# zai-org/SCAIL

Measured on AMD Instinct MI355X. Metric: denoising-step latent tokens/sec, higher is better.
Workload: dtype bf16

## Files before the change

include/scail_dit.h:

```cpp
#ifndef SCAIL_DIT_H
#define SCAIL_DIT_H

#include "scail_hip.h"

#ifdef __cplusplus
extern "C" {
#endif

typedef struct scail_dit_config {
    int32_t hidden_size;
    int32_t num_heads;
    int32_t inner_hidden_size;
    int32_t num_layers;
    int32_t text_dim;
    int32_t clip_dim;
    int32_t time_freq_dim;
    int32_t time_embed_dim;
    float layernorm_epsilon;
} scail_dit_config;

typedef struct scail_dit_layer {
    const scail_bf16* qkv_w; const float* qkv_b;
    const scail_bf16* o_w; const float* o_b;
    const float* qn; const float* kn;
// ... 11 lines not shown
    const scail_bf16* time0_w; const float* time0_b;
    const scail_bf16* time2_w; const float* time2_b;
    const scail_bf16* adaln_w; const float* adaln_b;
    const float* adaln_tables;
    const float* final_table;
    const scail_bf16* final_w; const float* final_b;
    const scail_dit_layer* layers;
} scail_dit_weights;

typedef struct scail_dit_cond {
    const scail_bf16* k_text;
    const scail_bf16* vt_text;
    const scail_bf16* k_clip;
    const scail_bf16* vt_clip;
    int64_t Lt, Lc, Bc;
} scail_dit_cond;

typedef struct scail_dit scail_dit;

int scail_dit_create(const scail_dit_config* cfg, const scail_dit_weights* w, scail_dit** out);
void scail_dit_destroy(scail_dit* h);

int64_t scail_dit_workspace_bytes(const scail_dit* h, int64_t B, int64_t T, int64_t H, int64_t W);

#define SCAIL_DIT_CFG_PAIR 1u
int scail_dit_step(scail_dit* h, const float* x, const float* timesteps, const scail_dit_cond* cond,
                   const scail_bf16* ref, int64_t n_ref, const scail_bf16* pose, int64_t n_pose,
                   const float* rope_cos, const float* rope_sin, float* out,
                   int64_t B, int64_t T, int64_t H, int64_t W, uint32_t flags, void* workspace, int64_t workspace_bytes, void* stream);

// ... 100 lines not shown
```

include/scail_hip.h:

```cpp
#ifndef SCAIL_HIP_H
#define SCAIL_HIP_H

#include <stdint.h>

#ifdef __cplusplus
extern "C" {
#endif

typedef uint16_t scail_bf16;

const char* scail_last_error(void);
int scail_abi_version(void);

enum {
    SCAIL_EPI_BIAS = 0,
    SCAIL_EPI_GELU_TANH = 1,
    SCAIL_EPI_GELU_ERF = 2,
    SCAIL_EPI_RESID = 3
};

int scail_gemm_bf16(const scail_bf16* x, int64_t lda, const scail_bf16* w, const float* bias,
                    scail_bf16* y, int64_t ldc, int64_t M, int64_t N, int64_t K, int epilogue,
                    const scail_bf16* resid, int64_t ldr, const float* gate, int64_t gate_stride,
                    int64_t rows_per_batch, void* stream);
// ... 56 lines not shown

int scail_flash_attn_rows_for(int64_t n_batch, int64_t heads, int64_t Lq);

int scail_flash_attn_count_restarts(uint32_t* device_counter);

int scail_cross_attn2_kernel_for(int64_t q_rs, int64_t k1_rs, int64_t k2_rs, int64_t o_rs, int64_t Lq, int64_t Lk1, int64_t Lk2,
                                 int64_t n_batch, int64_t heads);
int scail_cross_attn2_kernel_name_for(int64_t q_rs, int64_t k1_rs, int64_t k2_rs, int64_t o_rs, int64_t Lq, int64_t Lk1, int64_t Lk2,
                                      int64_t n_batch, int64_t heads, char* buf, int64_t len, int64_t* workgroups);
int scail_cross_attn2_bf16(const scail_bf16* q, int64_t q_bs, int64_t q_rs,
                           const scail_bf16* k1, int64_t k1_bs, int64_t k1_rs, const scail_bf16* vt1, int64_t vt1_bs, int64_t Lk1,
                           const scail_bf16* k2, int64_t k2_bs, int64_t k2_rs, const scail_bf16* vt2, int64_t vt2_bs, int64_t Lk2,
                           scail_bf16* o, int64_t o_bs, int64_t o_rs,
                           int64_t n_batch, int64_t heads, int64_t Lq, float scale, void* stream);

int scail_timestep_embedding(const float* t, float* out, int64_t n, int64_t dim, void* stream);

int scail_small_linear(const float* x, const scail_bf16* w, const float* b, float* y, int64_t M,
                       int64_t N, int64_t K, int act_in, int act_out, void* stream);

int scail_adaln_table(const float* emb, const float* table, float* out, int64_t n_layers,
                      int64_t n_batch, int64_t width, void* stream);

int scail_patchify(const float* x, const scail_bf16* ref, const scail_bf16* pose, scail_bf16* tok,
                   int64_t n_batch, int64_t n_ref, int64_t n_pose, int64_t T, int64_t H, int64_t W,
                   int64_t kpad, void* stream);

int scail_patchify_chars(const float* x, const scail_bf16* ref, const scail_bf16* pose, scail_bf16* tok,
                         int64_t n_batch, int64_t n_ref, int64_t n_pose, int64_t n_char, int64_t T, int64_t H, int64_t W,
                         int64_t kpad, void* stream);
// ... 98 lines not shown
```

scail_amd/csrc/attn.hip:

```cpp
#include <algorithm>
#include <atomic>
#include <cstring>
#include "common.h"

#define HD 128
#define QBLK 256
#define KVBLK 64
#define ATT_THREADS 512
#define K_LD (HD + 8)
#define V_LD (KVBLK + 8)
#define ATT_LDS_BYTES (2 * (KVBLK * K_LD + HD * V_LD) * 2)
#define ATT_PP_LDS_BYTES (ATT_LDS_BYTES + QBLK * K_LD * 2)

struct AttnParams {
    const u16* q; int64_t q_bs, q_rs;
    const u16* k; int64_t k_ss, k_bs, k_rs;
    const u16* vt; int64_t vt_ss, vt_bs;
    u16* o; int64_t o_bs, o_rs;
    int heads, Lq, Lk, Lkp, n_seg;
    float sl2;
    int accumulate;
    int probe;
};

// ... 243 lines not shown
    }
    if (p.probe && tid == 0) {
        atomicAdd(&g_attn_clk[0], (unsigned long long)__builtin_amdgcn_s_memtime() - clk0);
        atomicAdd(&g_attn_clk[1], 1ull);
    }
}


struct Cross2Params {
    const u16* q; int64_t q_bs, q_rs;
    const u16* k0; int64_t k0_bs, k0_rs; const u16* vt0; int64_t vt0_bs; int Lk0, Lkp0;
    const u16* k1; int64_t k1_bs, k1_rs; const u16* vt1; int64_t vt1_bs; int Lk1, Lkp1;
    u16* o; int64_t o_bs, o_rs;
    int heads, Lq;
    float sl2;
};

#define X2_THREADS 256
#define X2_LDS_BYTES (2 * (KVBLK * HD + HD * KVBLK) * 2)
__global__ __launch_bounds__(X2_THREADS, 2) void cross_attn2_kernel(Cross2Params p) {
    extern __shared__ __attribute__((aligned(16))) u16 smem[];
    u16* Ks = smem;
    u16* Vs = smem + 2 * KVBLK * HD;

    const int tid = threadIdx.x, lane = tid & 63;
    const int wave = __builtin_amdgcn_readfirstlane(tid >> 6);
    const int ql = lane & 31, g = lane >> 5;
    const int h = blockIdx.y;
    const int64_t b = blockIdx.z;
    const int q0 = blockIdx.x * 128 + wave * 32;

    bf16x8 qf[HD / 16];
    {
        const int qrow = min(q0 + ql, p.Lq - 1);
        const u16* qp = p.q + b * p.q_bs + (int64_t)qrow * p.q_rs + (int64_t)h * HD + g * 8;
#pragma unroll
        for (int ks = 0; ks < HD / 16; ++ks) qf[ks] = *reinterpret_cast<const bf16x8*>(qp + ks * 16);
    }

    const int dk_row = lane >> 4, dk_c = lane & 15, dv_row = lane >> 3, dv_c = lane & 7;
    const u16* kb0 = p.k0 + b * p.k0_bs + (int64_t)h * HD;
    const u16* kb1 = p.k1 + b * p.k1_bs + (int64_t)h * HD;
    const u16* vb0 = p.vt0 + b * p.vt0_bs + (int64_t)h * HD * p.Lkp0;
    const u16* vb1 = p.vt1 + b * p.vt1_bs + (int64_t)h * HD * p.Lkp1;
    const int n0 = p.Lkp0 / KVBLK, n1 = p.Lkp1 / KVBLK, ntiles = n0 + n1;
#define X2_ISSUE(tt_, buf_)                                                                                 \
    {                                                                                                       \
        const bool s1_ = (tt_) >= n0;                                                                       \
        const int key0_ = ((tt_) - (s1_ ? n0 : 0)) * KVBLK;                                                 \
        const u16* kp_ = s1_ ? kb1 : kb0;                                                                   \
        const int64_t krs_ = s1_ ? p.k1_rs : p.k0_rs;                                                       \
        const int last_ = (s1_ ? p.Lk1 : p.Lk0) - 1;                                                        \
        const int lkp_ = s1_ ? p.Lkp1 : p.Lkp0;                                                             \
        const u16* vp_ = (s1_ ? vb1 : vb0) + key0_;                                                         \
        _Pragma("unroll") for (int i_ = 0; i_ < 4; ++i_) {                                                  \
            const int j_ = wave * 4 + i_;                                                                   \
            const int kr_ = 4 * j_ + dk_row;                                                                \
            const u16* ks_src = kp_ + (int64_t)min(key0_ + kr_, last_) * krs_ + ((dk_c ^ (kr_ & 15)) << 3); \
            __builtin_amdgcn_global_load_lds((const __attribute__((address_space(1))) void*)ks_src,          \
                (__attribute__((address_space(3))) void*)(Ks + ((buf_) * KVBLK + 4 * j_) * HD), 16, 0, 0);   \
            const int vr_ = 8 * j_ + dv_row;                                                                \
            const u16* vs_src = vp_ + (int64_t)vr_ * lkp_ + ((dv_c ^ ((vr_ >> 1) & 7)) << 3);               \
            __builtin_amdgcn_global_load_lds((const __attribute__((address_space(1))) void*)vs_src,          \
                (__attribute__((address_space(3))) void*)(Vs + ((buf_) * HD + 8 * j_) * KVBLK), 16, 0, 0);   \
        }                                                                                                   \
    }
    int koff[HD / 16], voff[4];
// ... 36 lines not shown
        for (int f = 0; f < 2; ++f)
#pragma unroll
            for (int e = 0; e < 16; ++e) s[f][e] = 0.f;
        const u16* ks_ = Ks + (cur * KVBLK + ql) * HD;
#pragma unroll
        for (int ks = 0; ks < HD / 16; ++ks) {
#pragma unroll
            for (int f = 0; f < 2; ++f) {
                const bf16x8 kf = *reinterpret_cast<const bf16x8*>(ks_ + f * 32 * HD + koff[ks]);
                s[f] = __builtin_amdgcn_mfma_f32_32x32x16_bf16(kf, qf[ks], s[f], 0, 0, 0);
            }
        }
        {
            const bool s1 = tt >= n0;
            const int t = tt - (s1 ? n0 : 0), ns = s1 ? n1 : n0;
            const int tail = (s1 ? p.Lk1 : p.Lk0) - (ns - 1) * KVBLK;
            if (t == ns - 1 && tail < KVBLK) {
#pragma unroll
                for (int f = 0; f < 2; ++f)
#pragma unroll
                    for (int r = 0; r < 16; ++r) {
                        const int key = 32 * f + (r & 3) + 8 * (r >> 2) + 4 * g;
                        if (key >= tail) s[f][r] = -INFINITY;
                    }
            }
        }
        float mx = s[0][0];
#pragma unroll
        for (int f = 0; f < 2; ++f)
#pragma unroll
            for (int r = 0; r < 16; ++r) mx = fmaxf(mx, s[f][r]);
// ... 685 lines not shown
    return cross_choose(q_rs, k1_rs, k2_rs, o_rs, Lq, Lk1, Lk2, n_batch, heads, false).generated ? 4 : 2;
}

extern "C" int scail_cross_attn2_kernel_name_for(int64_t q_rs, int64_t k1_rs, int64_t k2_rs, int64_t o_rs, int64_t Lq, int64_t Lk1, int64_t Lk2,
                                                 int64_t n_batch, int64_t heads, char* buf, int64_t len, int64_t* workgroups) {
    SCAIL_REQUIRE(buf != nullptr, "null argument");
    SCAIL_REQUIRE(n_batch >= 1 && heads >= 1 && Lq >= 1 && Lk1 >= 1 && Lk2 >= 1, "need at least one pair, one query and one key per set");
    const CrossChoice c = cross_choose(q_rs, k1_rs, k2_rs, o_rs, Lq, Lk1, Lk2, n_batch, heads, workgroups != nullptr);
    if (c.grid < 0) return 2;
    SCAIL_REQUIRE((int64_t)std::strlen(c.name) < len, "buffer too small");
    std::strcpy(buf, c.name);
    if (workgroups != nullptr) *workgroups = c.grid;
    return 0;
}

extern "C" int scail_cross_attn2_bf16(const scail_bf16* q, int64_t q_bs, int64_t q_rs,
                                      const scail_bf16* k1, int64_t k1_bs, int64_t k1_rs, const scail_bf16* vt1, int64_t vt1_bs, int64_t Lk1,
                                      const scail_bf16* k2, int64_t k2_bs, int64_t k2_rs, const scail_bf16* vt2, int64_t vt2_bs, int64_t Lk2,
                                      scail_bf16* o, int64_t o_bs, int64_t o_rs,
                                      int64_t n_batch, int64_t heads, int64_t Lq, float scale, void* stream) {
    SCAIL_REQUIRE(Lk1 >= 1 && Lk2 >= 1 && Lk1 < (1ll << 30) && Lk2 < (1ll << 30), "cross_attn2: each key set needs at least one key");
    SCAIL_REQUIRE(heads >= 1 && heads < 65536 && n_batch < 65536 && Lq < (1ll << 31) - 256, "cross_attn2: grid limits");
    SCAIL_REQUIRE(q_rs % 8 == 0 && k1_rs % 8 == 0 && k2_rs % 8 == 0 && o_rs % 4 == 0 && q_bs % 8 == 0 && k1_bs % 8 == 0 && k2_bs % 8 == 0 &&
                      vt1_bs % 8 == 0 && vt2_bs % 8 == 0 && o_bs % 4 == 0,
                  "cross_attn2: strides must keep 16-byte (q, k, vt) / 8-byte (o) alignment");
    SCAIL_REQUIRE((reinterpret_cast<uintptr_t>(q) & 15) == 0 && (reinterpret_cast<uintptr_t>(k1) & 15) == 0 && (reinterpret_cast<uintptr_t>(k2) & 15) == 0 &&
                      (reinterpret_cast<uintptr_t>(vt1) & 15) == 0 && (reinterpret_cast<uintptr_t>(vt2) & 15) == 0 && (reinterpret_cast<uintptr_t>(o) & 7) == 0,
                  "cross_attn2: pointer alignment");
    if (n_batch == 0 || Lq == 0) return 0;
    const bool prescaled = scale == SCAIL_ATTN_Q_PRESCALED;
    SCAIL_REQUIRE(prescaled || (scale > 0.0f && scale < 3.0e38f), "cross_attn2: scale must be a positive finite number or SCAIL_ATTN_Q_PRESCALED");
    const CrossChoice c = cross_choose(q_rs, k1_rs, k2_rs, o_rs, Lq, Lk1, Lk2, n_batch, heads, true);
    if (c.generated) {
        hipFunction_t fn;
        if (int rc = scail_module_function("attn4", k_attn4_hsaco, c.name, &fn)) return rc;
// ... 3 lines not shown
        a.base.sl2 = prescaled ? 0.0f : scale * 1.4426950408889634f;
        a.base.thr = g_attn4_thr_log2;
        a.base.restarts = nullptr;
        a.k2 = k2; a.vt2 = vt2; a.k2_bs = k2_bs; a.vt2_bs = vt2_bs; a.Lk2 = (int32_t)Lk2; a.Lkp2 = (int32_t)((Lk2 + 63) / 64 * 64);
        a.n_wgs = (int32_t)c.grid;
        a.pad = 0;
        return scail_module_launch("cross_attn2 (attn4_x2)", fn, (unsigned)a.n_wgs, 256, a, stream);
    }
    Cross2Params p;
    p.q = q; p.q_bs = q_bs; p.q_rs = q_rs;
    p.k0 = k1; p.k0_bs = k1_bs; p.k0_rs = k1_rs; p.vt0 = vt1; p.vt0_bs = vt1_bs; p.Lk0 = (int)Lk1; p.Lkp0 = (int)((Lk1 + KVBLK - 1) / KVBLK * KVBLK);
    p.k1 = k2; p.k1_bs = k2_bs; p.k1_rs = k2_rs; p.vt1 = vt2; p.vt1_bs = vt2_bs; p.Lk1 = (int)Lk2; p.Lkp1 = (int)((Lk2 + KVBLK - 1) / KVBLK * KVBLK);
    p.o = o; p.o_bs = o_bs; p.o_rs = o_rs;
    p.heads = (int)heads; p.Lq = (int)Lq;
    p.sl2 = prescaled ? 1.0f : scale * 1.44269504088896340736f;
    const dim3 grid((unsigned)((Lq + 127) / 128), (unsigned)heads, (unsigned)n_batch);
    return scail_launch_lds<cross_attn2_kernel>("cross_attn2", X2_LDS_BYTES, grid, dim3(X2_THREADS), X2_LDS_BYTES, stream, p);
}
```

scail_amd/csrc/dit_step.hip:

```cpp
#include <algorithm>
#include <array>
#include <cmath>
#include <vector>

#include "common.h"
int scail_attn4_preload();
void scail_attn4_rows_hint(int rows);
int scail_gemm4_preload();
#include "../../include/scail_dit.h"

constexpr int PROF_CATS = 5;
struct ProfPool {
    std::vector<hipEvent_t> ev;
    size_t used = 0;
};

struct scail_dit {
    scail_dit_config cfg;
    scail_dit_weights w;
    std::vector<scail_dit_layer> layers;
    bool prof = false;
    ProfPool pool[PROF_CATS];
    hipEvent_t sp_ev[3] = {nullptr, nullptr, nullptr};
    uint32_t* restart_ctr = nullptr;
// ... 263 lines not shown
                           void* stream) {
    const scail_dit_config& c = h->cfg;
    const int64_t D = c.hidden_size, FF = c.inner_hidden_size, nh = c.num_heads;
    const float eps = c.layernorm_epsilon;
    const int64_t Ltp = (cond->Lt + 63) / 64 * 64, Lcp = (cond->Lc + 63) / 64 * 64;
    const int64_t M = nb * rpb;
    const scail_dit_layer& lw = h->layers[i];
    DIT_TRY(scail_layernorm_affine(hid, D, xn, D, lw.ln_w, lw.ln_b, M, D, eps, stream));
    DIT_PROF(SCAIL_DIT_PROF_GEMM, dit_gemm(h, i, G_CQ, bf, xn, D, lw.cq_b, q3, 3 * D, M, D, D, SCAIL_EPI_BIAS, nullptr, 0, nullptr, 0, 0, stream));
    DIT_TRY(scail_rmsnorm_rope_scaled(q3, 3 * D, q3, 3 * D, lw.cqn, nullptr, nullptr, M, M, D, 128, eps, ATTN_LOG2_SCALE, stream));
    const bool shared_clip = cond->Bc == 1;
    const scail_bf16* kt = cond->k_text + (i * Btot + b0) * cond->Lt * D;
    const scail_bf16* vtt = cond->vt_text + (i * Btot + b0) * nh * 128 * Ltp;
    const scail_bf16* kc = cond->k_clip + (i * cond->Bc + (shared_clip ? 0 : b0)) * cond->Lc * D;
    const scail_bf16* vtc = cond->vt_clip + (i * cond->Bc + (shared_clip ? 0 : b0)) * nh * 128 * Lcp;
    DIT_PROF(SCAIL_DIT_PROF_CROSS_ATTN, scail_cross_attn2_bf16(q3, rpb * 3 * D, 3 * D, kt, cond->Lt * D, D, vtt, nh * 128 * Ltp, cond->Lt,
                                                               kc, shared_clip ? 0 : cond->Lc * D, D, vtc, shared_clip ? 0 : nh * 128 * Lcp, cond->Lc,
                                                               att, rpb * D, D, nb, nh, rpb, SCAIL_ATTN_Q_PRESCALED, stream));
    DIT_PROF(SCAIL_DIT_PROF_GEMM, dit_gemm(h, i, G_CO, bf, att, D, lw.co_b, hid, D, M, D, D, SCAIL_EPI_RESID, hid, D, nullptr, 0, 0, stream));
    DIT_TRY(scail_ln_modulate(hid, D, xn, D, m + 3 * D, m + 4 * D, 6 * D, nb, rpb, rpb, 0, D, eps, stream));
    DIT_PROF(SCAIL_DIT_PROF_GEMM, dit_gemm(h, i, G_W1, bf, xn, D, lw.b1, ff, FF, M, FF, D, SCAIL_EPI_GELU_TANH, nullptr, 0, nullptr, 0, 0, stream));
    DIT_PROF(SCAIL_DIT_PROF_GEMM, dit_gemm(h, i, G_W2, bf, ff, FF, lw.b2, hid, D, M, D, FF, SCAIL_EPI_RESID, hid, D, m + 5 * D, 6 * D, rpb, stream));
    return 0;
}
static int block_tail(scail_dit* h, int64_t i, scail_bf16* hid, const float* m, const scail_dit_cond* cond, int64_t B, int64_t Ltok,
                      const BlockBufs& bf, int64_t row0, int64_t rows, bool pair, void* stream) {
    const int64_t D = h->cfg.hidden_size;
    scail_bf16 *att = bf.att, *q = bf.qkv, *xn = bf.xn, *ff = bf.ff;
    if (pair) {
        DIT_TRY(block_attn_out(h, i, hid + row0 * D, att + row0 * D, m, 1, rows, bf, stream));
        if (hipMemcpyAsync(hid + Ltok * D, hid, (size_t)Ltok * D * 2, hipMemcpyDeviceToDevice, (hipStream_t)stream) != hipSuccess) {
            scail_set_error("scail_dit (cfg pair): hipMemcpyAsync failed");
            return 2;
// ... 647 lines not shown
```

scail_amd/csrc/rowops.hip:

```cpp
#include "common.h"
#include <algorithm>
#include <atomic>
#include <cstring>

#define ROW_THREADS 256
#define ROW_MAXV 3

template <int MODE>
__global__ __launch_bounds__(ROW_THREADS) void ln_kernel(
    const u16* __restrict__ x, int64_t ldx, u16* __restrict__ y, int64_t ldy,
    const float* __restrict__ p0, const float* __restrict__ p1, int64_t mod_stride,
    int64_t rows_out, int64_t src_rows_per_batch, int64_t src_row_offset, int D, float eps) {
    __shared__ float red[4];
    const int64_t r = blockIdx.x;
    const int64_t b = r / rows_out;
    const int64_t i = r - b * rows_out;
    const u16* xr = x + (b * src_rows_per_batch + src_row_offset + i) * ldx;
    u16* yr = y + r * ldy;
    const int nvec = D >> 3;
    float v[ROW_MAXV][8];
    float s = 0.f;
#pragma unroll
    for (int j = 0; j < ROW_MAXV; ++j) {
        const int c = threadIdx.x + j * ROW_THREADS;
// ... 1044 lines not shown
    if (n == 0) return 0;
    hipLaunchKernelGGL(mul_bf16_kernel, dim3((unsigned)((n / 8 + 255) / 256)), dim3(256), 0, (hipStream_t)stream, a, b, y, n / 8);
    return scail_check_launch("mul_bf16");
}

extern "C" int scail_row_affine(const scail_bf16* x, scail_bf16* y, const float* rowscale, const scail_bf16* addrow, int64_t add_rows,
                                int64_t rows, int64_t D, void* stream) {
    SCAIL_REQUIRE(D % 8 == 0, "D must be a multiple of 8");
    if (rows == 0) return 0;
    const int64_t total = rows * (D / 8);
    hipLaunchKernelGGL(row_affine_kernel, dim3((unsigned)((total + 255) / 256)), dim3(256), 0, (hipStream_t)stream, x, y, rowscale,
                       addrow, add_rows > 0 ? add_rows : 1, rows, (int)(D / 8));
    return scail_check_launch("row_affine");
}

__global__ __launch_bounds__(256) void comm_standin_kernel(const uint4* __restrict__ src, uint4* __restrict__ dst, int64_t n16, int64_t min_ticks) {
    const int64_t t0 = (int64_t)wall_clock64();
    for (int64_t i = (int64_t)blockIdx.x * 256 + threadIdx.x; i < n16; i += (int64_t)gridDim.x * 256) dst[i] = src[i];
    while ((int64_t)wall_clock64() - t0 < min_ticks) __builtin_amdgcn_s_sleep(64);
}
extern "C" int scail_comm_standin(const void* src, void* dst, int64_t bytes, int32_t workgroups, int64_t min_ns, void* stream) {
    SCAIL_REQUIRE(bytes >= 0 && bytes % 16 == 0 && aligned16(src) && aligned16(dst), "bytes must be a multiple of 16, pointers 16-byte aligned");
    SCAIL_REQUIRE(workgroups >= 1 && workgroups <= 4096 && min_ns >= 0 && min_ns <= 1000000000ll, "workgroups in [1, 4096], min_ns in [0, 1e9]");
    hipLaunchKernelGGL(comm_standin_kernel, dim3((unsigned)workgroups), dim3(256), 0, (hipStream_t)stream,
                       reinterpret_cast<const uint4*>(src), reinterpret_cast<uint4*>(dst), bytes / 16, min_ns / 10);
    return scail_check_launch("comm_standin");
}
```

scail_amd/cstep.py:

```python
from __future__ import annotations

import ctypes as C
from typing import Dict

import torch

from . import lib as L

_p, _i64 = C.c_void_p, C.c_int64


class DitConfig(C.Structure):
    _fields_ = [("hidden_size", C.c_int32), ("num_heads", C.c_int32), ("inner_hidden_size", C.c_int32),
                ("num_layers", C.c_int32), ("text_dim", C.c_int32), ("clip_dim", C.c_int32),
                ("time_freq_dim", C.c_int32), ("time_embed_dim", C.c_int32), ("layernorm_epsilon", C.c_float)]


_LAYER_FIELDS = ["qkv_w", "qkv_b", "o_w", "o_b", "qn", "kn", "cq_w", "cq_b", "co_w", "co_b", "cqn", "ln_w", "ln_b",
                 "w1", "b1", "w2", "b2"]


class DitLayer(C.Structure):
    _fields_ = [(n, _p) for n in _LAYER_FIELDS]


class DitWeights(C.Structure):
    _fields_ = [(n, _p) for n in ("patch_w", "patch_b", "pose_w", "pose_b", "time0_w", "time0_b", "time2_w", "time2_b",
                                  "adaln_w", "adaln_b", "adaln_tables", "final_table", "final_w", "final_b")] + \
               [("layers", C.POINTER(DitLayer))]


class DitCond(C.Structure):
    _fields_ = [("k_text", _p), ("vt_text", _p), ("k_clip", _p), ("vt_clip", _p), ("Lt", _i64), ("Lc", _i64), ("Bc", _i64)]


EXCHANGE_FN = C.CFUNCTYPE(C.c_int, C.c_void_p, C.c_int32, C.c_int32, C.c_int32, C.c_void_p)
SP_ALLGATHER, SP_ULYSSES = 0, 1
SP_FWD_START, SP_FWD_WAIT, SP_BACK_START, SP_BACK_WAIT = 0, 1, 2, 3


class DitSp(C.Structure):
    _fields_ = [("ranks", C.c_int32), ("mode", C.c_int32), ("send", _p), ("recv", _p), ("ofull", _p), ("back", _p),
                ("exchange", EXCHANGE_FN), ("user", _p), ("side_stream", _p * 2)]


def _cond_struct(cond: Dict) -> "DitCond":
    k_text, k_clip = cond["k_text"], cond["k_clip"]
    return DitCond(k_text.data_ptr(), cond["vt_text"].data_ptr(), k_clip.data_ptr(), cond["vt_clip"].data_ptr(),
                   k_text.shape[2], k_clip.shape[2], k_clip.shape[1])


class CStep:

    def __init__(self, net, W: Dict):
        L.load()
        self._keep = W
        cfg = DitConfig(net.hidden_size, net.num_attention_heads, net.inner_hidden_size, net.num_layers, net.text_dim,
                        1280, net.time_freq_dim, net.time_embed_dim, float(net.layernorm_epsilon))
        layers = (DitLayer * net.num_layers)()
        for i, lw in enumerate(W["layers"]):
            for n in _LAYER_FIELDS:
                setattr(layers[i], n, lw[n].data_ptr())
        w = DitWeights(W["patch_w"].data_ptr(), W["patch_b"].data_ptr(), W["pose_w"].data_ptr(), W["pose_b"].data_ptr(),
                       W["time_embed.0.w"].data_ptr(), W["time_embed.0.b"].data_ptr(),
# ... 196 lines not shown
```

scail_amd/dit.py:

```python
from __future__ import annotations

import os

import math
from functools import reduce
from operator import mul
from typing import Dict, Optional

import torch
from torch import nn

from . import lib as L
from . import ops, rope

_STR2DTYPE = {"fp32": torch.float32, "fp16": torch.float16, "bf16": torch.bfloat16}


def _get(args, name, default=None):
    if args is None:
        return default
    if isinstance(args, dict):
        return args.get(name, default)
    return getattr(args, name, default)

# ... 166 lines not shown
        self.gemm_precision, self.fp8_mask = _fp8_options(gemm_precision, fp8_gemms)
        self.fp8_scaling = _fp8_scaling_option(fp8_scaling, self.gemm_precision)
        self.fp8_layer_masks = _fp8_layer_options(fp8_layers, num_layers, self.fp8_mask)
        self.fp8_probe_table = None
        if self.fp8_mask:
            D, FF = self.hidden_size, self.inner_hidden_size
            for name, (n, k) in (("qkv", (3 * D, D)), ("o", (D, D)), ("cq", (D, D)), ("co", (D, D)), ("w1", (FF, D)), ("w2", (D, FF))):
                if self.fp8_mask & L.FP8_GEMMS[name] and (n % 128 or k % 128):
                    raise NotImplementedError(f"fp8 GEMM {name} ({n} x {k}): the fp8 kernel needs N and K multiples of 128")
        self._build_params(device, init_seed)
        self._prepared: Optional[Dict] = None
        self._cond_cache = None
        self._rope_cache: Dict = {}
        self._ws: Dict = {}
        self.cache_conditioning = True
        self.sp = None
        self._tap = None
        self.kernel_timer = None
        self.use_c_step = os.environ.get("SCAIL_C_STEP", "1") != "0"
        self._cstep = None
        self._c_blocks = False

    def param_spec(self) -> Dict[str, tuple]:
        D, FF, Dt = self.hidden_size, self.inner_hidden_size, self.time_embed_dim
        s: Dict[str, tuple] = {}
        s["mixins.patch_embed.proj.weight"] = (D, 20, 1, 2, 2)
        s["mixins.patch_embed.proj.bias"] = (D,)
        s["mixins.patch_embed.proj_pose.weight"] = (D, 20, 1, 2, 2)
        s["mixins.patch_embed.proj_pose.bias"] = (D,)
        for i in range(self.num_layers):
# ... 166 lines not shown
        Ltp, Lcp = (Lt + 63) // 64 * 64, (Lc + 63) // 64 * 64
        nl = self.num_layers
        k_text = torch.empty(nl, B, Lt, D, device=dev, dtype=torch.bfloat16)
        vt_text = torch.empty(nl, B, H, 128, Ltp, device=dev, dtype=torch.bfloat16)
        k_clip = torch.empty(nl, Bc, Lc, D, device=dev, dtype=torch.bfloat16)
        vt_clip = torch.empty(nl, Bc, H, 128, Lcp, device=dev, dtype=torch.bfloat16)
        kv = torch.empty(B, Lt, 2 * D, device=dev, dtype=torch.bfloat16)
        kvc = torch.empty(Bc, Lc, 2 * D, device=dev, dtype=torch.bfloat16)
        for i, lw in enumerate(W["layers"]):
            ops.gemm(text, lw["ckv_w"], lw["ckv_b"], out=kv)
            ops.rmsnorm_rope(kv[..., :D], lw["ckn"], out=k_text[i], eps=self.layernorm_epsilon)
            ops.transpose_v(kv[..., D:], H, out=vt_text[i])
            ops.gemm(cl, lw["clipkv_w"], lw["clipkv_b"], out=kvc)
            ops.rmsnorm_rope(kvc[..., :D], lw["clipkn"], out=k_clip[i], eps=self.layernorm_epsilon)
            ops.transpose_v(kvc[..., D:], H, out=vt_clip[i])
        return dict(k_text=k_text, vt_text=vt_text, k_clip=k_clip, vt_clip=vt_clip)

    def _timed(self, tag, fn, *a, **k):
        if self.kernel_timer is None:
            return fn(*a, **k)
        return self.kernel_timer.run(tag, fn, *a, **k)

    def _rope(self, T, Hp, Wp, H_shift, W_shift, device, n_char=1):
        key = (T, Hp, Wp, H_shift, W_shift, n_char)
        if key not in self._rope_cache:
            mt = (self.num_frames - 1) // self.time_compressed_rate + 1
            cos, sin = rope.build_tables(self.head_dim, T, Hp, Wp, H_shift, W_shift, self.global_rope_H,
                                         self.global_rope_W, max_T=mt, max_H=self.latent_height // 2,
                                         max_W=self.latent_width // 2 + 120, n_char=n_char)
            self._rope_cache[key] = (cos.to(device), sin.to(device))
        return self._rope_cache[key]
# ... 172 lines not shown
            sh_m, sc_m, g_m = m[:, 3 * D:4 * D], m[:, 4 * D:5 * D], m[:, 5 * D:6 * D]
            ops.ln_modulate(h, sh_a, sc_a, out=xn, eps=eps)
            if sp is None:
                ops.gemm(xn, lw["qkv_w"], lw["qkv_b"], out=qkv)
                ops.rmsnorm_rope(k, lw["kn"], cos, sin, rows_per_batch=Ltok, eps=eps)
                ops.transpose_v(v, nh, out=vt)
                ops.rmsnorm_rope(q, lw["qn"], cos, sin, rows_per_batch=Ltok, eps=eps, out_scale=ops.ATTN_LOG2_SCALE)
                self._timed("self_attn", ops.flash_attn, q, k, vt, out=att, q_prescaled=True)
            else:
                sp.self_attention(self, lw, xn, qkv, vt, cos, sin, att, Ltok, eps)
            ops.gemm(att, lw["o_w"], lw["o_b"], out=h, epilogue=L.EPI_RESID, resid=h, gate=g_a, rows_per_batch=Ltok)
            ops.layernorm_affine(h, lw["ln_w"], lw["ln_b"], out=xn, eps=eps)
            cq = qkv[..., :D]
            ops.gemm(xn, lw["cq_w"], lw["cq_b"], out=cq)
            ops.rmsnorm_rope(cq, lw["cqn"], eps=eps, out_scale=ops.ATTN_LOG2_SCALE)
            ops.cross_attn2(cq, cond["k_text"][i], cond["vt_text"][i], cond["k_clip"][i], cond["vt_clip"][i], out=att, q_prescaled=True)
            ops.gemm(att, lw["co_w"], lw["co_b"], out=h, epilogue=L.EPI_RESID, resid=h)
            ops.ln_modulate(h, sh_m, sc_m, out=xn, eps=eps)
            ops.gemm(xn, lw["w1"], lw["b1"], out=ff, epilogue=L.EPI_GELU_TANH)
            ops.gemm(ff, lw["w2"], lw["b2"], out=h, epilogue=L.EPI_RESID, resid=h, gate=g_m, rows_per_batch=Ltok)
            if self._tap is not None:
                self._tap(i, h)

        ops.ln_modulate(h, fin[:, :D], fin[:, D:], out=ws["xf"], eps=eps, rows_out=Lnoise, src_row_offset=Lref)
        ops.gemm(ws["xf"], W["final_w"], W["final_b"], out=ws["tokout"])
        return ops.unpatchify(ws["tokout"], T, H, Wd)
```

scail_amd/lib.py:

```python
from __future__ import annotations

import ctypes as C
import os

_HERE = os.path.dirname(os.path.abspath(__file__))
LIB_PATH = os.path.join(_HERE, "libscail_hip_abl.so" if os.environ.get("SCAIL_ABLATIONS", "0") not in ("", "0") else "libscail_hip.so")

_p = C.c_void_p
_i64 = C.c_int64
_i = C.c_int
_f = C.c_float

SIGNATURES = {
    "scail_gemm_bf16": [_p, _i64, _p, _p, _p, _i64, _i64, _i64, _i64, _i, _p, _i64, _p, _i64, _i64, _p],
    "scail_ln_modulate": [_p, _i64, _p, _i64, _p, _p, _i64, _i64, _i64, _i64, _i64, _i64, _f, _p],
    "scail_layernorm_affine": [_p, _i64, _p, _i64, _p, _p, _i64, _i64, _f, _p],
    "scail_rmsnorm_rope": [_p, _i64, _p, _i64, _p, _p, _p, _i64, _i64, _i64, _i64, _f, _p],
    "scail_rmsnorm_rope_scaled": [_p, _i64, _p, _i64, _p, _p, _p, _i64, _i64, _i64, _i64, _f, _f, _p],
    "scail_rmsnorm_rope_slabs": [_p, _i64, _p, _i64, _i64, _i64, _p, _p, _p, _i64, _i64, _i64, _i64, _f, _f, _p],
    "scail_row_kernel_name_for": [_i, _i64, _i64, _i64, _i64, _p, _i64, _p],
    "scail_slabs_to_rows": [_p, _i64, _i64, _p, _i64, _i64, _i64, _p],
    "scail_transpose_v": [_p, _i64, _i64, _p, _i64, _i64, _i64, _i64, _p],
    "scail_flash_attn_bf16": [_p, _i64, _i64, _p, _i64, _i64, _i64, _p, _i64, _i64, _p, _i64, _i64,
                              _i64, _i64, _i64, _i64, _i64, _f, _i, _p],
    "scail_flash_attn_kernel_for": [_i64, _i64, _i64, _i64, _i64, _i, _i],
    "scail_flash_attn_kernel_name_for": [_i64, _i64, _i64, _i64, _i64, _i64, _i64, _i, _i, _p, _i64, _p],
    "scail_flash_attn_rows_for": [_i64, _i64, _i64],
    "scail_flash_attn_count_restarts": [_p],
    "scail_comm_standin": [_p, _p, _i64, C.c_int32, _i64, _p],
    "scail_cross_attn2_kernel_for": [_i64, _i64, _i64, _i64, _i64, _i64, _i64, _i64, _i64],
    "scail_cross_attn2_kernel_name_for": [_i64, _i64, _i64, _i64, _i64, _i64, _i64, _i64, _i64, _p, _i64, _p],
    "scail_gemm_kernel_for": [_i64, _i64, _i64, _i64, _i64, _i64, _i],
    "scail_gemm_kernel_name_for": [_i64, _i64, _i64, _i64, _i64, _i64, _i, _i, _p, _i64],
    "scail_conv3d_kernel_for": [_p, _i64, _i64, _i],
    "scail_conv3d_norm_fused_for": [_p, _i64],
    "scail_conv3d_kernel_name_for": [_p, _i64, _i64, _i, _p, _i64],
    "scail_cross_attn2_bf16": [_p, _i64, _i64, _p, _i64, _i64, _p, _i64, _i64, _p, _i64, _i64, _p, _i64, _i64, _p, _i64, _i64,
                               _i64, _i64, _i64, _f, _p],
    "scail_timestep_embedding": [_p, _p, _i64, _i64, _p],
    "scail_small_linear": [_p, _p, _p, _p, _i64, _i64, _i64, _i, _i, _p],
    "scail_adaln_table": [_p, _p, _p, _i64, _i64, _i64, _p],
    "scail_patchify": [_p, _p, _p, _p, _i64, _i64, _i64, _i64, _i64, _i64, _i64, _p],
    "scail_patchify_chars": [_p, _p, _p, _p, _i64, _i64, _i64, _i64, _i64, _i64, _i64, _i64, _p],
    "scail_unpatchify": [_p, _p, _i64, _i64, _i64, _i64, _p],
    "scail_cfg_euler": [_p, _p, _i64, _f, _f, _p],
    "scail_tile_gather": [_p, _p, _p, _i64, _i64, _i64, _p],
    "scail_tile_blend_acc": [_p, _p, _p, _p, _i64, _i64, _i64, _f, _p],
    "scail_tile_finish": [_p, _p, _p, _i64, _i64, _f, _p],
    "scail_conv3d_cl": [_p, _p, _p, _p, _i64, _p, _i64, _p, _p],
    "scail_conv3d_cl_norm": [_p, _p, _p, _p, _i64, _p, _p, _p],
    "scail_conv3d_cl_resid_norm": [_p, _p, _p, _p, _p, _i64, _p, _i64, _p, _p, _p],
    "scail_rms_silu": [_p, _p, _p, _i64, _i64, _i, _p],
    "scail_softmax_rows": [_p, _i64, _i64, _i64, _f, _p],
# ... 134 lines not shown
```

scail_amd/ops.py:

```python
from __future__ import annotations

import math
from typing import Optional

import torch

from . import lib as L

bf16 = torch.bfloat16
f32 = torch.float32


def _stream() -> int:
    return torch.cuda.current_stream().cuda_stream


def _chk(t: torch.Tensor, dtype, name: str):
    if not t.is_cuda:
        raise L.ScailHipError(f"{name}: tensor must be on the GPU (scail_amd has no CPU path)")
    if t.dtype != dtype:
        raise L.ScailHipError(f"{name}: expected {dtype}, got {t.dtype}")


def _ptr(t: Optional[torch.Tensor]) -> Optional[int]:
# ... 241 lines not shown
        out = torch.empty(B, Lq, D, device=q.device, dtype=bf16)
    _chk(out, bf16, "flash_attn.out")
    assert out.stride(2) == 1
    k_bs = 0 if (k_broadcast or k.shape[0] == 1) else k.stride(0)
    vt_bs = 0 if (k_broadcast or vt.shape[0] == 1) else vt.stride(0)
    if scale is None:
        scale = 1.0 / math.sqrt(128)
    if q_prescaled:
        scale = ATTN_Q_PRESCALED
    L.call("scail_flash_attn_bf16", q.data_ptr(), q.stride(0), q.stride(1), k.data_ptr(), k_seg_stride, k_bs,
           k.stride(1), vt.data_ptr(), vt_seg_stride, vt_bs, out.data_ptr(), out.stride(0), out.stride(1), B, H, Lq,
           Lk, n_seg, scale, 1 if accumulate else 0, _stream())
    return out


def cross_attn2(q, k1, vt1, k2, vt2, out=None, scale=None, q_prescaled=False):
    _chk(q, bf16, "cross_attn2.q")
    B, Lq, D = q.shape
    H = D // 128
    assert D == H * 128 and q.stride(2) == 1
    if out is None:
        out = torch.empty(B, Lq, D, device=q.device, dtype=bf16)
    _chk(out, bf16, "cross_attn2.out")
    assert out.stride(2) == 1 and out.shape == (B, Lq, D)
    sets = []
    for k, vt in ((k1, vt1), (k2, vt2)):
        _chk(k, bf16, "cross_attn2.k"); _chk(vt, bf16, "cross_attn2.vt")
        Lk = k.shape[1]
        assert k.shape[0] in (1, B) and vt.shape[0] == k.shape[0] and k.shape[2] == D and k.stride(2) == 1
        assert vt.shape[1:] == (H, 128, (Lk + 63) // 64 * 64) and vt[0].is_contiguous(), (vt.shape, Lk)
        sets += [k.data_ptr(), 0 if k.shape[0] == 1 else k.stride(0), k.stride(1), vt.data_ptr(), 0 if vt.shape[0] == 1 else vt.stride(0), Lk]
    if scale is None:
        scale = 1.0 / math.sqrt(128)
    if q_prescaled:
        scale = ATTN_Q_PRESCALED
    L.call("scail_cross_attn2_bf16", q.data_ptr(), q.stride(0), q.stride(1), *sets, out.data_ptr(), out.stride(0), out.stride(1),
           B, H, Lq, scale, _stream())
    return out


def timestep_embedding(t, dim):
    _chk(t, f32, "timestep_embedding.t")
    out = torch.empty(t.shape[0], dim, device=t.device, dtype=f32)
    L.call("scail_timestep_embedding", t.data_ptr(), out.data_ptr(), t.shape[0], dim, _stream())
    return out


def small_linear(x, w, b=None, act_in=L.ACT_NONE, act_out=L.ACT_NONE):
    _chk(x, f32, "small_linear.x"); _chk(w, bf16, "small_linear.w")
    assert x.is_contiguous() and w.is_contiguous()
# ... 358 lines not shown
```

Measured before the change: 9164.

## Collapse trailing identical text keys into one weighted key in cross-attention

Adds a key-run scan that finds the trailing run of text keys whose K and V are identical to the last key (for example padding tokens), and records the effective key count plus log2 of the run length. Cross-attention then visits only the tiles up to that point and adds the log2 weight to the last key's score, which is mathematically equivalent to attending to every duplicate. This cuts K/V loads and score work for padded text conditioning. It adds a scan pass per conditioning build, which is cached across steps, and relies on the query being prescaled into log2 units.

```diff
diff --git a/include/scail_dit.h b/include/scail_dit.h
--- a/include/scail_dit.h
+++ b/include/scail_dit.h
@@ -49,6 +49,7 @@
     const scail_bf16* k_clip;
     const scail_bf16* vt_clip;
     int64_t Lt, Lc, Bc;
+    const scail_key_run_rec* text_runs;
 } scail_dit_cond;
 
 typedef struct scail_dit scail_dit;
diff --git a/include/scail_hip.h b/include/scail_hip.h
--- a/include/scail_hip.h
+++ b/include/scail_hip.h
@@ -94,6 +94,15 @@
                            scail_bf16* o, int64_t o_bs, int64_t o_rs,
                            int64_t n_batch, int64_t heads, int64_t Lq, float scale, void* stream);
 
+typedef struct scail_key_run_rec { int32_t n_eff; float lg; } scail_key_run_rec;
+int scail_key_run(const scail_bf16* k, int64_t k_bs, int64_t k_rs, const scail_bf16* vt, int64_t vt_bs, int64_t Lk,
+                  int64_t n_batch, int64_t heads, scail_key_run_rec* records, void* stream);
+int scail_cross_attn2_run_bf16(const scail_bf16* q, int64_t q_bs, int64_t q_rs,
+                               const scail_bf16* k1, int64_t k1_bs, int64_t k1_rs, const scail_bf16* vt1, int64_t vt1_bs, int64_t Lk1,
+                               const scail_bf16* k2, int64_t k2_bs, int64_t k2_rs, const scail_bf16* vt2, int64_t vt2_bs, int64_t Lk2,
+                               scail_bf16* o, int64_t o_bs, int64_t o_rs,
+                               int64_t n_batch, int64_t heads, int64_t Lq, float scale, const scail_key_run_rec* runs, void* stream);
+
 int scail_timestep_embedding(const float* t, float* out, int64_t n, int64_t dim, void* stream);
 
 int scail_small_linear(const float* x, const scail_bf16* w, const float* b, float* y, int64_t M,
diff --git a/scail_amd/csrc/attn.hip b/scail_amd/csrc/attn.hip
--- a/scail_amd/csrc/attn.hip
+++ b/scail_amd/csrc/attn.hip
@@ -281,6 +281,7 @@
     u16* o; int64_t o_bs, o_rs;
     int heads, Lq;
     float sl2;
+    const int32_t* run;
 };
 
 #define X2_THREADS 256
@@ -310,14 +311,20 @@
     const u16* kb1 = p.k1 + b * p.k1_bs + (int64_t)h * HD;
     const u16* vb0 = p.vt0 + b * p.vt0_bs + (int64_t)h * HD * p.Lkp0;
     const u16* vb1 = p.vt1 + b * p.vt1_bs + (int64_t)h * HD * p.Lkp1;
-    const int n0 = p.Lkp0 / KVBLK, n1 = p.Lkp1 / KVBLK, ntiles = n0 + n1;
+    int lk0 = p.Lk0;
+    float lg = 0.f;
+    if (p.run != nullptr) {
+        lk0 = min(max(__builtin_amdgcn_readfirstlane(p.run[2 * b]), 1), p.Lk0);
+        lg = __int_as_float(__builtin_amdgcn_readfirstlane(p.run[2 * b + 1]));
+    }
+    const int n0 = (lk0 + KVBLK - 1) / KVBLK, n1 = p.Lkp1 / KVBLK, ntiles = n0 + n1;
 #define X2_ISSUE(tt_, buf_)                                                                                 \
     {                                                                                                       \
         const bool s1_ = (tt_) >= n0;                                                                       \
         const int key0_ = ((tt_) - (s1_ ? n0 : 0)) * KVBLK;                                                 \
         const u16* kp_ = s1_ ? kb1 : kb0;                                                                   \
         const int64_t krs_ = s1_ ? p.k1_rs : p.k0_rs;                                                       \
-        const int last_ = (s1_ ? p.Lk1 : p.Lk0) - 1;                                                        \
+        const int last_ = (s1_ ? p.Lk1 : lk0) - 1;                                                          \
         const int lkp_ = s1_ ? p.Lkp1 : p.Lkp0;                                                             \
         const u16* vp_ = (s1_ ? vb1 : vb0) + key0_;                                                         \
         _Pragma("unroll") for (int i_ = 0; i_ < 4; ++i_) {                                                  \
@@ -384,7 +391,16 @@
         {
             const bool s1 = tt >= n0;
             const int t = tt - (s1 ? n0 : 0), ns = s1 ? n1 : n0;
-            const int tail = (s1 ? p.Lk1 : p.Lk0) - (ns - 1) * KVBLK;
+            const int tail = (s1 ? p.Lk1 : lk0) - (ns - 1) * KVBLK;
+            if (p.run != nullptr && tt == n0 - 1) {
+#pragma unroll
+                for (int f = 0; f < 2; ++f)
+#pragma unroll
+                    for (int r = 0; r < 16; ++r) {
+                        const int key = 32 * f + (r & 3) + 8 * (r >> 2) + 4 * g;
+                        if (key == tail - 1) s[f][r] += lg;
+                    }
+            }
             if (t == ns - 1 && tail < KVBLK) {
 #pragma unroll
                 for (int f = 0; f < 2; ++f)
@@ -1100,11 +1116,11 @@
     return 0;
 }
 
-extern "C" int scail_cross_attn2_bf16(const scail_bf16* q, int64_t q_bs, int64_t q_rs,
-                                      const scail_bf16* k1, int64_t k1_bs, int64_t k1_rs, const scail_bf16* vt1, int64_t vt1_bs, int64_t Lk1,
-                                      const scail_bf16* k2, int64_t k2_bs, int64_t k2_rs, const scail_bf16* vt2, int64_t vt2_bs, int64_t Lk2,
-                                      scail_bf16* o, int64_t o_bs, int64_t o_rs,
-                                      int64_t n_batch, int64_t heads, int64_t Lq, float scale, void* stream) {
+static int cross_attn2_launch(const scail_bf16* q, int64_t q_bs, int64_t q_rs,
+                              const scail_bf16* k1, int64_t k1_bs, int64_t k1_rs, const scail_bf16* vt1, int64_t vt1_bs, int64_t Lk1,
+                              const scail_bf16* k2, int64_t k2_bs, int64_t k2_rs, const scail_bf16* vt2, int64_t vt2_bs, int64_t Lk2,
+                              scail_bf16* o, int64_t o_bs, int64_t o_rs,
+                              int64_t n_batch, int64_t heads, int64_t Lq, float scale, const void* runs, void* stream) {
     SCAIL_REQUIRE(Lk1 >= 1 && Lk2 >= 1 && Lk1 < (1ll << 30) && Lk2 < (1ll << 30), "cross_attn2: each key set needs at least one key");
     SCAIL_REQUIRE(heads >= 1 && heads < 65536 && n_batch < 65536 && Lq < (1ll << 31) - 256, "cross_attn2: grid limits");
     SCAIL_REQUIRE(q_rs % 8 == 0 && k1_rs % 8 == 0 && k2_rs % 8 == 0 && o_rs % 4 == 0 && q_bs % 8 == 0 && k1_bs % 8 == 0 && k2_bs % 8 == 0 &&
@@ -1138,6 +1154,31 @@
     p.o = o; p.o_bs = o_bs; p.o_rs = o_rs;
     p.heads = (int)heads; p.Lq = (int)Lq;
     p.sl2 = prescaled ? 1.0f : scale * 1.44269504088896340736f;
+    p.run = static_cast<const int32_t*>(runs);
     const dim3 grid((unsigned)((Lq + 127) / 128), (unsigned)heads, (unsigned)n_batch);
     return scail_launch_lds<cross_attn2_kernel>("cross_attn2", X2_LDS_BYTES, grid, dim3(X2_THREADS), X2_LDS_BYTES, stream, p);
 }
+
+extern "C" int scail_cross_attn2_bf16(const scail_bf16* q, int64_t q_bs, int64_t q_rs,
+                                      const scail_bf16* k1, int64_t k1_bs, int64_t k1_rs, const scail_bf16* vt1, int64_t vt1_bs, int64_t Lk1,
+                                      const scail_bf16* k2, int64_t k2_bs, int64_t k2_rs, const scail_bf16* vt2, int64_t vt2_bs, int64_t Lk2,
+                                      scail_bf16* o, int64_t o_bs, int64_t o_rs,
+                                      int64_t n_batch, int64_t heads, int64_t Lq, float scale, void* stream) {
+    return cross_attn2_launch(q, q_bs, q_rs, k1, k1_bs, k1_rs, vt1, vt1_bs, Lk1, k2, k2_bs, k2_rs, vt2, vt2_bs, Lk2, o, o_bs, o_rs, n_batch, heads,
+                              Lq, scale, nullptr, stream);
+}
+
+extern "C" int scail_cross_attn2_run_bf16(const scail_bf16* q, int64_t q_bs, int64_t q_rs,
+                                          const scail_bf16* k1, int64_t k1_bs, int64_t k1_rs, const scail_bf16* vt1, int64_t vt1_bs, int64_t Lk1,
+                                          const scail_bf16* k2, int64_t k2_bs, int64_t k2_rs, const scail_bf16* vt2, int64_t vt2_bs, int64_t Lk2,
+                                          scail_bf16* o, int64_t o_bs, int64_t o_rs,
+                                          int64_t n_batch, int64_t heads, int64_t Lq, float scale, const scail_key_run_rec* runs, void* stream) {
+    if (scale != SCAIL_ATTN_Q_PRESCALED) {
+        scail_set_error("scail_cross_attn2_run_bf16: the scale must be SCAIL_ATTN_Q_PRESCALED (a run's log2 weight is exact only on scores in "
+                        "log2 units), got " + std::to_string(scale));
+        return 1;
+    }
+    SCAIL_REQUIRE((reinterpret_cast<uintptr_t>(runs) & 7) == 0, "cross_attn2: the run records must be 8-byte aligned");
+    return cross_attn2_launch(q, q_bs, q_rs, k1, k1_bs, k1_rs, vt1, vt1_bs, Lk1, k2, k2_bs, k2_rs, vt2, vt2_bs, Lk2, o, o_bs, o_rs, n_batch, heads,
+                              Lq, scale, runs, stream);
+}
diff --git a/scail_amd/csrc/dit_step.hip b/scail_amd/csrc/dit_step.hip
--- a/scail_amd/csrc/dit_step.hip
+++ b/scail_amd/csrc/dit_step.hip
@@ -301,9 +301,10 @@
     const scail_bf16* vtt = cond->vt_text + (i * Btot + b0) * nh * 128 * Ltp;
     const scail_bf16* kc = cond->k_clip + (i * cond->Bc + (shared_clip ? 0 : b0)) * cond->Lc * D;
     const scail_bf16* vtc = cond->vt_clip + (i * cond->Bc + (shared_clip ? 0 : b0)) * nh * 128 * Lcp;
-    DIT_PROF(SCAIL_DIT_PROF_CROSS_ATTN, scail_cross_attn2_bf16(q3, rpb * 3 * D, 3 * D, kt, cond->Lt * D, D, vtt, nh * 128 * Ltp, cond->Lt,
-                                                               kc, shared_clip ? 0 : cond->Lc * D, D, vtc, shared_clip ? 0 : nh * 128 * Lcp, cond->Lc,
-                                                               att, rpb * D, D, nb, nh, rpb, SCAIL_ATTN_Q_PRESCALED, stream));
+    const scail_key_run_rec* runs = cond->text_runs == nullptr ? nullptr : cond->text_runs + (i * Btot + b0);
+    DIT_PROF(SCAIL_DIT_PROF_CROSS_ATTN, scail_cross_attn2_run_bf16(q3, rpb * 3 * D, 3 * D, kt, cond->Lt * D, D, vtt, nh * 128 * Ltp, cond->Lt,
+                                                                   kc, shared_clip ? 0 : cond->Lc * D, D, vtc, shared_clip ? 0 : nh * 128 * Lcp, cond->Lc,
+                                                                   att, rpb * D, D, nb, nh, rpb, SCAIL_ATTN_Q_PRESCALED, runs, stream));
     DIT_PROF(SCAIL_DIT_PROF_GEMM, dit_gemm(h, i, G_CO, bf, att, D, lw.co_b, hid, D, M, D, D, SCAIL_EPI_RESID, hid, D, nullptr, 0, 0, stream));
     DIT_TRY(scail_ln_modulate(hid, D, xn, D, m + 3 * D, m + 4 * D, 6 * D, nb, rpb, rpb, 0, D, eps, stream));
     DIT_PROF(SCAIL_DIT_PROF_GEMM, dit_gemm(h, i, G_W1, bf, xn, D, lw.b1, ff, FF, M, FF, D, SCAIL_EPI_GELU_TANH, nullptr, 0, nullptr, 0, 0, stream));
diff --git a/scail_amd/csrc/rowops.hip b/scail_amd/csrc/rowops.hip
--- a/scail_amd/csrc/rowops.hip
+++ b/scail_amd/csrc/rowops.hip
@@ -1082,6 +1082,109 @@
     return scail_check_launch("row_affine");
 }
 
+static_assert(sizeof(scail_key_run_rec) == 8 && offsetof(scail_key_run_rec, lg) == 4, "scail_key_run_rec is {int32 n_eff; float lg}");
+
+__global__ __launch_bounds__(256) void key_run_scan_kernel(const u16* __restrict__ k, int64_t k_bs, int64_t k_rs, const u16* __restrict__ vt,
+                                                           int64_t vt_bs, int Lk, int Lkp, int D, scail_key_run_rec* rec) {
+    __shared__ int red[4];
+    const int64_t b = blockIdx.y;
+    const int tid = threadIdx.x;
+    const int64_t stride = (int64_t)gridDim.x * 256;
+    int worst = 0;
+    const u16* kb = k + b * k_bs;
+    const u16* klast = kb + (int64_t)(Lk - 1) * k_rs;
+    const int dc = D / 8;
+    const int64_t nk = (int64_t)(Lk - 1) * dc;
+    for (int64_t i = (int64_t)blockIdx.x * 256 + tid; i < nk; i += stride) {
+        const int j = (int)(i / dc), c = (int)(i - (int64_t)j * dc);
+        const uint4 a = *reinterpret_cast<const uint4*>(kb + (int64_t)j * k_rs + c * 8);
+        const uint4 r = *reinterpret_cast<const uint4*>(klast + c * 8);
+        if (a.x != r.x || a.y != r.y || a.z != r.z || a.w != r.w) worst = max(worst, j + 1);
+    }
+    const u16* vb = vt + b * vt_bs;
+    const int vc = (Lk + 15) / 16 * 2;
+    const int plast = ((Lk - 1) & ~12) | ((((Lk - 1) >> 3) & 1) << 2) | ((((Lk - 1) >> 2) & 1) << 3);
+    const int64_t nv = (int64_t)D * vc;
+    for (int64_t i = (int64_t)blockIdx.x * 256 + tid; i < nv; i += stride) {
+        const int row = (int)(i / vc), c = (int)(i - (int64_t)row * vc);
+        const u16* vr = vb + (int64_t)row * Lkp;
+        const uint4 a = *reinterpret_cast<const uint4*>(vr + c * 8);
+        const uint32_t ref = vr[plast];
+        const uint32_t w[4] = {a.x, a.y, a.z, a.w};
+#pragma unroll
+        for (int e = 0; e < 8; ++e) {
+            const int col = c * 8 + e;
+            const int key = (col & ~12) | (((col >> 3) & 1) << 2) | (((col >> 2) & 1) << 3);
+            const uint32_t v = (w[e >> 1] >> (16 * (e & 1))) & 0xffffu;
+            if (key < Lk - 1 && v != ref) worst = max(worst, key + 1);
+        }
+    }
+#pragma unroll
+    for (int off = 32; off > 0; off >>= 1) worst = max(worst, __shfl_xor(worst, off, 64));
+    if ((tid & 63) == 0) red[tid >> 6] = worst;
+    __syncthreads();
+    if (tid == 0) {
+        worst = max(max(red[0], red[1]), max(red[2], red[3]));
+        if (worst > 0) atomicMax(&rec[b].n_eff, worst);
+    }
+}
+
+__global__ void key_run_finish_kernel(scail_key_run_rec* rec, int Lk, int n_batch) {
+    const int b = blockIdx.x * 256 + threadIdx.x;
+    if (b >= n_batch) return;
+    const int r = rec[b].n_eff;
+    const int n = Lk - r;
+    scail_key_run_rec out;
+    out.n_eff = r + 1;
+    out.lg = (n & (n - 1)) == 0 ? (float)(__ffs(n) - 1) : (float)log2((double)n);
+    rec[b] = out;
+}
+
+extern "C" int scail_key_run(const scail_bf16* k, int64_t k_bs, int64_t k_rs, const scail_bf16* vt, int64_t vt_bs, int64_t Lk,
+                             int64_t n_batch, int64_t heads, scail_key_run_rec* records, void* stream) {
+    if (k == nullptr || vt == nullptr || records == nullptr) {
+        scail_set_error(std::string("scail_key_run: null pointer (") + (k == nullptr ? "k" : vt == nullptr ? "vt" : "records") + ")");
+        return 1;
+    }
+    if (Lk < 1 || Lk >= (1ll << 30)) {
+        scail_set_error("scail_key_run: a key set needs 1 .. 2^30 - 1 keys, got Lk = " + std::to_string(Lk));
+        return 1;
+    }
+    if (heads < 1 || heads >= 65536 || n_batch < 0 || n_batch >= 65536) {
+        scail_set_error("scail_key_run: heads must be 1 .. 65535 and n_batch 0 .. 65535, got heads = " + std::to_string(heads) + ", n_batch = " +
+                        std::to_string(n_batch));
+        return 1;
+    }
+    const int64_t D = heads * 128, Lkp = (Lk + 63) / 64 * 64;
+    if (k_rs < D) {
+        scail_set_error("scail_key_run: the K row stride is shorter than a row of heads * 128 = " + std::to_string(D) + " elements, got k_rs = " +
+                        std::to_string(k_rs));
+        return 1;
+    }
+    if (n_batch > 1 && (k_bs < D || vt_bs < D * Lkp)) {
+        scail_set_error("scail_key_run: a batch stride is shorter than its data (K: a row of " + std::to_string(D) + ", V^T: heads * 128 * ceil64(Lk) = " +
+                        std::to_string(D * Lkp) + " elements), got k_bs = " + std::to_string(k_bs) + ", vt_bs = " + std::to_string(vt_bs));
+        return 1;
+    }
+    SCAIL_REQUIRE(k_rs % 8 == 0 && k_bs % 8 == 0 && vt_bs % 8 == 0 && aligned16(k) && aligned16(vt), "16-byte alignment");
+    SCAIL_REQUIRE((reinterpret_cast<uintptr_t>(records) & 7) == 0, "the records must be 8-byte aligned");
+    if (n_batch == 0) return 0;
+    const hipError_t e = hipMemsetAsync(records, 0, (size_t)n_batch * sizeof(scail_key_run_rec), (hipStream_t)stream);
+    if (e != hipSuccess) {
+        scail_set_error(std::string("scail_key_run: hipMemsetAsync failed: ") + hipGetErrorString(e));
+        return 2;
+    }
+    if (Lk > 1) {
+        const int64_t chunks = (Lk - 1) * (D / 8) + D * ((Lk + 15) / 16 * 2);
+        const unsigned blocks = (unsigned)std::min<int64_t>(std::max<int64_t>((chunks + 1023) / 1024, 1), 1024);
+        hipLaunchKernelGGL(key_run_scan_kernel, dim3(blocks, (unsigned)n_batch), dim3(256), 0, (hipStream_t)stream, k, k_bs, k_rs, vt, vt_bs, (int)Lk,
+                           (int)Lkp, (int)D, records);
+        if (int rc = scail_check_launch("key_run (scan)")) return rc;
+    }
+    hipLaunchKernelGGL(key_run_finish_kernel, dim3((unsigned)((n_batch + 255) / 256)), dim3(256), 0, (hipStream_t)stream, records, (int)Lk, (int)n_batch);
+    return scail_check_launch("key_run");
+}
+
 __global__ __launch_bounds__(256) void comm_standin_kernel(const uint4* __restrict__ src, uint4* __restrict__ dst, int64_t n16, int64_t min_ticks) {
     const int64_t t0 = (int64_t)wall_clock64();
     for (int64_t i = (int64_t)blockIdx.x * 256 + threadIdx.x; i < n16; i += (int64_t)gridDim.x * 256) dst[i] = src[i];
diff --git a/scail_amd/cstep.py b/scail_amd/cstep.py
--- a/scail_amd/cstep.py
+++ b/scail_amd/cstep.py
@@ -31,7 +31,8 @@
 
 
 class DitCond(C.Structure):
-    _fields_ = [("k_text", _p), ("vt_text", _p), ("k_clip", _p), ("vt_clip", _p), ("Lt", _i64), ("Lc", _i64), ("Bc", _i64)]
+    _fields_ = [("k_text", _p), ("vt_text", _p), ("k_clip", _p), ("vt_clip", _p), ("Lt", _i64), ("Lc", _i64), ("Bc", _i64),
+                ("text_runs", _p)]
 
 
 EXCHANGE_FN = C.CFUNCTYPE(C.c_int, C.c_void_p, C.c_int32, C.c_int32, C.c_int32, C.c_void_p)
@@ -47,7 +48,8 @@
 def _cond_struct(cond: Dict) -> "DitCond":
     k_text, k_clip = cond["k_text"], cond["k_clip"]
     return DitCond(k_text.data_ptr(), cond["vt_text"].data_ptr(), k_clip.data_ptr(), cond["vt_clip"].data_ptr(),
-                   k_text.shape[2], k_clip.shape[2], k_clip.shape[1])
+                   k_text.shape[2], k_clip.shape[2], k_clip.shape[1],
+                   cond["text_runs"].data_ptr() if cond.get("text_runs") is not None else None)
 
 
 class CStep:
diff --git a/scail_amd/dit.py b/scail_amd/dit.py
--- a/scail_amd/dit.py
+++ b/scail_amd/dit.py
@@ -204,6 +204,8 @@
         self._rope_cache: Dict = {}
         self._ws: Dict = {}
         self.cache_conditioning = True
+        self.text_runs = True
+        self.text_runs_min_keys = 65
         self.sp = None
         self._tap = None
         self.kernel_timer = None
@@ -400,7 +402,8 @@
             ops.gemm(cl, lw["clipkv_w"], lw["clipkv_b"], out=kvc)
             ops.rmsnorm_rope(kvc[..., :D], lw["clipkn"], out=k_clip[i], eps=self.layernorm_epsilon)
             ops.transpose_v(kvc[..., D:], H, out=vt_clip[i])
-        return dict(k_text=k_text, vt_text=vt_text, k_clip=k_clip, vt_clip=vt_clip)
+        text_runs = ops.key_run(k_text, vt_text) if self.text_runs and Lt >= self.text_runs_min_keys else None
+        return dict(k_text=k_text, vt_text=vt_text, k_clip=k_clip, vt_clip=vt_clip, text_runs=text_runs)
 
     def _timed(self, tag, fn, *a, **k):
         if self.kernel_timer is None:
@@ -603,7 +606,9 @@
             cq = qkv[..., :D]
             ops.gemm(xn, lw["cq_w"], lw["cq_b"], out=cq)
             ops.rmsnorm_rope(cq, lw["cqn"], eps=eps, out_scale=ops.ATTN_LOG2_SCALE)
-            ops.cross_attn2(cq, cond["k_text"][i], cond["vt_text"][i], cond["k_clip"][i], cond["vt_clip"][i], out=att, q_prescaled=True)
+            runs = cond.get("text_runs")
+            ops.cross_attn2(cq, cond["k_text"][i], cond["vt_text"][i], cond["k_clip"][i], cond["vt_clip"][i], out=att, q_prescaled=True,
+                            runs=None if runs is None else runs[i])
             ops.gemm(att, lw["co_w"], lw["co_b"], out=h, epilogue=L.EPI_RESID, resid=h)
             ops.ln_modulate(h, sh_m, sc_m, out=xn, eps=eps)
             ops.gemm(xn, lw["w1"], lw["b1"], out=ff, epilogue=L.EPI_GELU_TANH)
diff --git a/scail_amd/lib.py b/scail_amd/lib.py
--- a/scail_amd/lib.py
+++ b/scail_amd/lib.py
@@ -37,6 +37,9 @@
     "scail_conv3d_kernel_name_for": [_p, _i64, _i64, _i, _p, _i64],
     "scail_cross_attn2_bf16": [_p, _i64, _i64, _p, _i64, _i64, _p, _i64, _i64, _p, _i64, _i64, _p, _i64, _i64, _p, _i64, _i64,
                                _i64, _i64, _i64, _f, _p],
+    "scail_cross_attn2_run_bf16": [_p, _i64, _i64, _p, _i64, _i64, _p, _i64, _i64, _p, _i64, _i64, _p, _i64, _i64, _p, _i64, _i64,
+                                   _i64, _i64, _i64, _f, _p, _p],
+    "scail_key_run": [_p, _i64, _i64, _p, _i64, _i64, _i64, _i64, _p, _p],
     "scail_timestep_embedding": [_p, _p, _i64, _i64, _p],
     "scail_small_linear": [_p, _p, _p, _p, _i64, _i64, _i64, _i, _i, _p],
     "scail_adaln_table": [_p, _p, _p, _i64, _i64, _i64, _p],
diff --git a/scail_amd/ops.py b/scail_amd/ops.py
--- a/scail_amd/ops.py
+++ b/scail_amd/ops.py
@@ -279,7 +279,21 @@
     return out
 
 
-def cross_attn2(q, k1, vt1, k2, vt2, out=None, scale=None, q_prescaled=False):
+def key_run(k, vt, out=None):
+    _chk(k, bf16, "key_run.k"); _chk(vt, bf16, "key_run.vt")
+    lead, Lk, D = k.shape[:-2], k.shape[-2], k.shape[-1]
+    H = D // 128
+    assert D == H * 128 and k.is_contiguous() and vt.is_contiguous() and vt.shape == (*lead, H, 128, (Lk + 63) // 64 * 64), (k.shape, vt.shape)
+    n = math.prod(lead)
+    if out is None:
+        out = torch.empty(*lead, 2, device=k.device, dtype=torch.int32)
+    _chk(out, torch.int32, "key_run.out")
+    assert out.is_contiguous() and out.shape == (*lead, 2)
+    L.call("scail_key_run", k.data_ptr(), Lk * D, D, vt.data_ptr(), D * vt.shape[-1], Lk, n, H, out.data_ptr(), _stream())
+    return out
+
+
+def cross_attn2(q, k1, vt1, k2, vt2, out=None, scale=None, q_prescaled=False, runs=None):
     _chk(q, bf16, "cross_attn2.q")
     B, Lq, D = q.shape
     H = D // 128
@@ -299,6 +313,12 @@
         scale = 1.0 / math.sqrt(128)
     if q_prescaled:
         scale = ATTN_Q_PRESCALED
+    if runs is not None:
+        _chk(runs, torch.int32, "cross_attn2.runs")
+        assert runs.shape == (B, 2) and runs.is_contiguous() and k1.shape[0] == B, (runs.shape, k1.shape)
+        L.call("scail_cross_attn2_run_bf16", q.data_ptr(), q.stride(0), q.stride(1), *sets, out.data_ptr(), out.stride(0), out.stride(1),
+               B, H, Lq, scale, runs.data_ptr(), _stream())
+        return out
     L.call("scail_cross_attn2_bf16", q.data_ptr(), q.stride(0), q.stride(1), *sets, out.data_ptr(), out.stride(0), out.stride(1),
            B, H, Lq, scale, _stream())
     return out
```

After: 9238 (median of 6 runs). Within noise of the previous version (+0.8%).
